# ukeSJTU/tiaozhanbei-unet

Measured on AMD Instinct MI355X. Metric: training images/sec, AnomalyUNet 256x256 bs=32 per GPU, higher is better.
Workload: dtype bf16; 1 GPU; AnomalyUNet 3x256x256, bs=32/GPU, MSE+focal loss, Adam (BASELINE.json configs[2], synthetic randn images, bernoulli masks); global_batch=32, parallelism=dp1, accumulate=fp32, master_params=fp32, dist_world=1, reserved_cus=0, cu_budget=256

## Files before the change

### tiaozhanbei_unet_amd/csrc/common.h

```cpp
#pragma once
#include <hip/hip_runtime.h>
#include <stdint.h>
#include <stdio.h>

#include "../../include/unet_hip.h"

typedef __bf16 bf16_t;
typedef __attribute__((ext_vector_type(8))) __bf16 bf16x8;
typedef __attribute__((ext_vector_type(4))) __bf16 bf16x4;
typedef __attribute__((ext_vector_type(4))) short s16x4;
typedef __attribute__((ext_vector_type(4))) float f32x4;
typedef __attribute__((ext_vector_type(16))) float f32x16;
typedef __attribute__((ext_vector_type(4))) uint32_t u32x4;
typedef __attribute__((ext_vector_type(2))) uint32_t u32x2;

#define WAVE 64

void unet_set_error(const char* fmt, ...);
int32_t unet_check_launch(const char* what);

#define UNET_REQUIRE(cond, code, ...)  \
  do {                                 \
    if (!(cond)) {                     \
      unet_set_error(__VA_ARGS__);     \
      return (code);                   \
    }                                  \
  } while (0)

int unet_cu_budget();
void unet_set_max_lds(const void* kernel, int bytes);

void unet_prof_begin(int kclass, hipStream_t s);
void unet_prof_end(int kclass, double flops, hipStream_t s, const char* kernel, double bytes);
struct ProfScope {
  int k; double f; hipStream_t s; const char* name;
  double bytes;
  ProfScope(int kclass, double flops, hipStream_t st, const char* kernel = nullptr, double alg_bytes = 0.0)
      : k(kclass), f(flops), s(st), name(kernel), bytes(alg_bytes) {
    unet_prof_begin(k, s);
  }
  ~ProfScope() { unet_prof_end(k, f, s, name, bytes); }
};

bool unet_internal_convt_gemm_ok(int mode, int dtype, int n, int h, int w, int c_in, int c_out);
int32_t unet_internal_convt_gemm(int mode, int n, int h, int w, const void* a, const void* w_packed, const float* bias,
                                 void* out, int c_in, int c_out, hipStream_t s);

int32_t unet_internal_colsum(int dtype, const void* x, int64_t pixels, int C, float* out, float* ws,
                              size_t ws_bytes, hipStream_t s);

int32_t unet_internal_bn_partials(int dtype, const void* y, int64_t pixels, int C, float* part, int* n_parts,
                                  hipStream_t s);

template <typename T> struct ET;
template <> struct ET<float> {
  static constexpr int ES = 4;
  static constexpr int PIECE = 4;
  static constexpr int KGC = 8;
  __device__ static inline float to_f(float v) { return v; }
  __device__ static inline float from_f(float v) { return v; }
};
template <> struct ET<bf16_t> {
  static constexpr int ES = 2;
  static constexpr int PIECE = 8;
  static constexpr int KGC = 16;
  __device__ static inline float to_f(bf16_t v) { return (float)v; }
  __device__ static inline bf16_t from_f(float v) { return (bf16_t)v; }
};

template <typename T> struct Vec;
template <> struct Vec<float> {
  static constexpr int N = 4;
  __device__ static inline void load(const float* p, float (&o)[4]) {
    f32x4 v = *reinterpret_cast<const f32x4*>(p);
    o[0] = v[0]; o[1] = v[1]; o[2] = v[2]; o[3] = v[3];
  }
  __device__ static inline void store(float* p, const float (&o)[4]) {
    f32x4 v = {o[0], o[1], o[2], o[3]};
    *reinterpret_cast<f32x4*>(p) = v;
  }
};
template <> struct Vec<bf16_t> {
  static constexpr int N = 8;
  __device__ static inline void load(const bf16_t* p, float (&o)[8]) {
    bf16x8 v = *reinterpret_cast<const bf16x8*>(p);
#pragma unroll
    for (int i = 0; i < 8; ++i) o[i] = (float)v[i];
  }
  __device__ static inline void store(bf16_t* p, const float (&o)[8]) {
    bf16x8 v;
#pragma unroll
    for (int i = 0; i < 8; ++i) v[i] = (bf16_t)o[i];
    *reinterpret_cast<bf16x8*>(p) = v;
  }
};

__host__ __device__ static inline int cdiv(int a, int b) { return (a + b - 1) / b; }
__host__ __device__ static inline int64_t cdiv64(int64_t a, int64_t b) { return (a + b - 1) / b; }

__device__ __forceinline__ uint32_t score_key(float x) {
  uint32_t u = __float_as_uint(x);
  if (u == 0x80000000u) u = 0u;
  return (u & 0x80000000u) ? ~u : (u | 0x80000000u);
}
__device__ __forceinline__ float score_of_key(uint32_t k) {
  return __uint_as_float((k & 0x80000000u) ? (k & 0x7fffffffu) : ~k);
}
__device__ __forceinline__ bool finite_score(float x) { return (__float_as_uint(x) & 0x7f800000u) != 0x7f800000u; }

__host__ __device__ static inline int unet_seg_col(int q, int split, int c) {
  if (split > 0 && q >= split) {
    const int p0 = (split + 63) / 64 * 64;
    if (q < p0) return -1;
    q = q - p0 + split;
  }
  return q < c ? q : -1;
}

__device__ static inline float unet_pack_seg_value(const float* __restrict__ w, int Co, int Ci, int rows, int K, int mode,
                                                   int split, long long i, const float* __restrict__ scale) {
  const int b = (int)(i % K);
  const long long t = i / K;
  const int a = (int)(t % rows), tap = (int)(t / rows);
  if (mode == UNET_PACK_CONV_FWD) {
    const int ci = unet_seg_col(b, split, Ci);
    return (a < Co && ci >= 0) ? w[((long long)a * Ci + ci) * 9 + tap] * (scale ? scale[a] : 1.f) : 0.f;
  }
  const int ci = unet_seg_col(a, split, Ci);
  return (b < Co && ci >= 0) ? w[((long long)b * Ci + ci) * 9 + (8 - tap)] : 0.f;
}
```

### tiaozhanbei_unet_amd/csrc/first.hip

```cpp
#include <stdlib.h>

#include <algorithm>

#include "conv_common.h"

namespace {

constexpr unsigned OOB = 0xFFFFFFF0u;
constexpr int FIRST_CO = 64;

struct SegPos { int seg, y, n; };
__device__ __forceinline__ SegPos seg_step(SegPos p, int dseg, int dy, int dn, int segs_row, int H) {
  p.seg += dseg;
  int c = p.seg >= segs_row;
  p.seg -= c ? segs_row : 0;
  p.y += dy + c;
  c = p.y >= H;
  p.y -= c ? H : 0;
  p.n += dn + c;
  return p;
}
struct SegWalk { SegPos first; int dseg, dy, dn; };
__device__ __forceinline__ SegWalk seg_walk(long long u0, long long stride, int segs_row, int H) {
  SegWalk w;
// ... 26 lines not shown
#pragma unroll
  for (int ct = 0; ct < 4; ++ct)
#pragma unroll
    for (int e = 0; e < 8; ++e) {
      const int k = kb * 8 + e;
      float v = 0.f;
      if (k < K) {
        const int tap = k / P.CI, ci = k - tap * P.CI;
        v = P.w[((ct * 16 + l15) * P.CI + ci) * 9 + tap];
      }
      wa[ct][e] = (bf16_t)v;
    }
  int rel[8], reli[8], dyv[8], dxv[8];
#pragma unroll
  for (int e = 0; e < 8; ++e) {
    const int k = kb * 8 + e;
    const int tap = k < K ? k / P.CI : 0, ci = k < K ? k - tap * P.CI : 0;
    dyv[e] = k < K ? tap / 3 - 1 : 1 << 20;
    dxv[e] = tap % 3 - 1;
    rel[e] = (ci * HW + dyv[e] * P.W + dxv[e]) * 4;
    reli[e] = k < K ? rel[e] : 0;
  }

  const int segs_row = P.W >> 4;
  const long long stride = (long long)gridDim.x * 4;
  const unsigned img_bytes = (unsigned)P.CI * HW * 4u;

  auto gather = [&](SegPos q, float (&xv)[8]) {
    const int x = q.seg * 16 + l15;
    const __amdgpu_buffer_rsrc_t rs =
        __builtin_amdgcn_make_buffer_rsrc((void*)(P.x + (size_t)q.n * P.CI * HW), (short)0, (int)img_bytes, 0x00020000);
    const int base = (q.y * P.W + x) * 4;
    if (q.y > 0 && q.y + 1 < P.H && q.seg > 0 && q.seg + 1 < segs_row) {
#pragma unroll
      for (int e = 0; e < 8; ++e)
        xv[e] = __builtin_bit_cast(float, __builtin_amdgcn_raw_buffer_load_b32(rs, (unsigned)(base + reli[e]), 0, 0));
    } else {
#pragma unroll
      for (int e = 0; e < 8; ++e) {
        const bool ok = (unsigned)(q.y + dyv[e]) < (unsigned)P.H && (unsigned)(x + dxv[e]) < (unsigned)P.W;
        xv[e] = __builtin_bit_cast(float, __builtin_amdgcn_raw_buffer_load_b32(rs, ok ? (unsigned)(base + rel[e]) : OOB, 0, 0));
      }
    }
  };

  float bs[4][4], bq[4][4];
#pragma unroll
  for (int ct = 0; ct < 4; ++ct)
#pragma unroll
    for (int j = 0; j < 4; ++j) { bs[ct][j] = 0.f; bq[ct][j] = 0.f; }

  constexpr int FU = 2;
  const int wave_u = __builtin_amdgcn_readfirstlane(wave);
  const SegWalk wk = seg_walk(((long long)blockIdx.x * 4 + wave_u) * FU, stride * FU, segs_row, P.H);
  SegPos cur = wk.first;
  float xc[FU][8], xn[FU][8];
#pragma unroll
  for (int i = 0; i < FU; ++i) {
    const SegPos q = seg_step(cur, i, 0, 0, segs_row, P.H);
    if (q.n < P.N) gather(q, xc[i]);
  }
  while (cur.n < P.N) {
    const SegPos nxt = seg_step(cur, wk.dseg, wk.dy, wk.dn, segs_row, P.H);
#pragma unroll
    for (int i = 0; i < FU; ++i) {
      const SegPos q = seg_step(nxt, i, 0, 0, segs_row, P.H);
      if (q.n < P.N) gather(q, xn[i]);
    }
#pragma unroll
    for (int i = 0; i < FU; ++i) {
      const SegPos q = seg_step(cur, i, 0, 0, segs_row, P.H);
      if (q.n >= P.N) break;
      bf16x8 fb;
#pragma unroll
      for (int e = 0; e < 8; ++e) fb[e] = (bf16_t)xc[i][e];
      f32x4 acc[4];
#pragma unroll
      for (int ct = 0; ct < 4; ++ct) {
        acc[ct] = f32x4{0.f, 0.f, 0.f, 0.f};
        acc[ct] = __builtin_amdgcn_mfma_f32_16x16x32_bf16(wa[ct], fb, acc[ct], 0, 0, 0);
      }
      const long long pix = ((long long)q.n * P.H + q.y) * P.W + q.seg * 16 + l15;
      bf16_t* orow = reinterpret_cast<bf16_t*>(P.y) + pix * FIRST_CO;
#pragma unroll
      for (int cp = 0; cp < 2; ++cp) {
        bf16x4 ra, rb;
#pragma unroll
        for (int j = 0; j < 4; ++j) { ra[j] = (bf16_t)acc[2 * cp][j]; rb[j] = (bf16_t)acc[2 * cp + 1][j]; }
#pragma unroll
        for (int j = 0; j < 4; ++j) {
          const float qa = (float)ra[j], qb = (float)rb[j];
          bs[2 * cp][j] += qa;      bq[2 * cp][j] = fmaf(qa, qa, bq[2 * cp][j]);
          bs[2 * cp + 1][j] += qb;  bq[2 * cp + 1][j] = fmaf(qb, qb, bq[2 * cp + 1][j]);
        }
        const u32x2 ua = __builtin_bit_cast(u32x2, ra), ub = __builtin_bit_cast(u32x2, rb);
        const auto s0 = __builtin_amdgcn_permlane16_swap(ua[0], ub[0], false, false);
        const auto s1 = __builtin_amdgcn_permlane16_swap(ua[1], ub[1], false, false);
        *reinterpret_cast<u32x4*>(orow + cp * 32 + (kb & 1) * 16 + (kb >> 1) * 8) = u32x4{s0[0], s1[0], s0[1], s1[1]};
      }
    }
#pragma unroll
    for (int i = 0; i < FU; ++i)
#pragma unroll
      for (int e = 0; e < 8; ++e) xc[i][e] = xn[i][e];
    cur = nxt;
  }

  if (P.part) {
    {
      float rv[32];
#pragma unroll
      for (int ct = 0; ct < 4; ++ct)
#pragma unroll
        for (int j = 0; j < 4; ++j) { rv[ct * 4 + j] = bs[ct][j]; rv[16 + ct * 4 + j] = bq[ct][j]; }
      row16_sum_n(rv);
#pragma unroll
      for (int ct = 0; ct < 4; ++ct)
#pragma unroll
        for (int j = 0; j < 4; ++j) { bs[ct][j] = rv[ct * 4 + j]; bq[ct][j] = rv[16 + ct * 4 + j]; }
    }
    if (l15 == 0) {
#pragma unroll
      for (int ct = 0; ct < 4; ++ct)
#pragma unroll
        for (int j = 0; j < 4; ++j) {
          red[wave][0][ct * 16 + kb * 4 + j] = bs[ct][j];
          red[wave][1][ct * 16 + kb * 4 + j] = bq[ct][j];
        }
    }
    __syncthreads();
    if (tid < 2 * FIRST_CO) {
      const int q = tid / FIRST_CO, c = tid - q * FIRST_CO;
      const float t = ((red[0][q][c] + red[1][q][c]) + red[2][q][c]) + red[3][q][c];
      P.part[((size_t)blockIdx.x * 2 + q) * FIRST_CO + c] = t;
    }
  }
}

__device__ inline bf16x8 tr_frag2(const char* base, int off0, int off1) {
  typedef __attribute__((address_space(3))) s16x4 lds_s16x4;
  s16x4 lo = __builtin_amdgcn_ds_read_tr16_b64_v4i16((lds_s16x4*)(base + off0));
  s16x4 hi = __builtin_amdgcn_ds_read_tr16_b64_v4i16((lds_s16x4*)(base + off1));
  typedef __attribute__((ext_vector_type(8))) short s16x8;
  s16x8 v = {lo[0], lo[1], lo[2], lo[3], hi[0], hi[1], hi[2], hi[3]};
  return __builtin_bit_cast(bf16x8, v);
}

template <bool BNB>
__global__ __launch_bounds__(256, BNB ? 2 : 4) void first_wgrad_kernel(const FirstParams P) {
  constexpr int SEGB = BNB ? 4096 : 2048;
  __shared__ __attribute__((aligned(16))) char smem[BNB ? 4 * 2 * 2 * 4096 : 4 * FIRST_CO * 32 * 4];
  typedef __attribute__((address_space(3))) void lds_void;
  const int tid = threadIdx.x, lane = tid & 63, wave = tid >> 6;
  const int l31 = lane & 31, hh = lane >> 5;
  const int K = 9 * P.CI;
  const int HW = P.H * P.W;
  constexpr int WU = 2;
  char* const wbuf = smem + wave * (WU * 2 * SEGB);

  const bool kvalid = l31 < K;
  const int tap = kvalid ? l31 / P.CI : 0, ci = kvalid ? l31 - tap * P.CI : 0;
  const int dy = tap / 3 - 1, dx = tap % 3 - 1;
  const int relb = (ci * HW + dy * P.W + dx + 8 * hh) * 4;

  const int g = lane >> 4, i16 = lane & 15;
  const int kq = 8 * (g >> 1) + (i16 >> 2);
  const int chb = (16 * (g & 1) + 4 * (i16 & 3)) * 2;
  const int swz = ((kq >> 1) & 1) << 2;
  int aoff[2];
#pragma unroll
  for (int wr = 0; wr < 2; ++wr) {
    const int cb = wr * 64 + chb;
    aoff[wr] = kq * 128 + ((((cb >> 4) ^ swz)) << 4) + (cb & 15);
  }
  unsigned dsrc[2];
#pragma unroll
  for (int i = 0; i < 2; ++i) {
    const int row = i * 8 + (lane >> 3), pp = lane & 7;
    dsrc[i] = (unsigned)(row * 128 + ((pp ^ (((row >> 1) & 1) << 2)) << 4));
  }

  const int segs_row = P.W >> 4;
  const long long stride = (long long)gridDim.x * 4;
  const unsigned img_bytes = (unsigned)P.CI * HW * 4u;
  const long long dy_total = (long long)P.N * HW * FIRST_CO * 2;
  auto issue = [&](SegPos q, int slot, float (&xv)[8]) {
    const int seg = q.seg, y = q.y, n = q.n;
    const long long pix0 = ((long long)n * P.H + y) * P.W + seg * 16;
    const __amdgpu_buffer_rsrc_t drs = __builtin_amdgcn_make_buffer_rsrc(
        (void*)(P.y + pix0 * (FIRST_CO * 2)), (short)0, (int)std::min<long long>(2048, dy_total - pix0 * (FIRST_CO * 2)),
        0x00020000);
#pragma unroll
    for (int i = 0; i < 2; ++i)
      __builtin_amdgcn_raw_ptr_buffer_load_lds(drs, (lds_void*)(wbuf + slot * SEGB + i * 1024), 16, dsrc[i], 0, 0, 0);
    if constexpr (BNB) {
      const __amdgpu_buffer_rsrc_t yrs = __builtin_amdgcn_make_buffer_rsrc(
          (void*)(P.y_raw + pix0 * (FIRST_CO * 2)), (short)0, (int)std::min<long long>(2048, dy_total - pix0 * (FIRST_CO * 2)),
          0x00020000);
#pragma unroll
      for (int i = 0; i < 2; ++i)
        __builtin_amdgcn_raw_ptr_buffer_load_lds(yrs, (lds_void*)(wbuf + slot * SEGB + 2048 + i * 1024), 16, dsrc[i], 0, 0, 0);
    }
    const __amdgpu_buffer_rsrc_t xrs =
        __builtin_amdgcn_make_buffer_rsrc((void*)(P.x + (size_t)n * P.CI * HW), (short)0, (int)img_bytes, 0x00020000);
    const int x0 = seg * 16;
    const int base = (y * P.W + x0) * 4 + relb;
    if (y > 0 && y + 1 < P.H && seg > 0 && seg + 1 < segs_row) {
      const unsigned b0 = kvalid ? (unsigned)base : 0u;
#pragma unroll
      for (int e = 0; e < 8; ++e)
        xv[e] = __builtin_bit_cast(float, __builtin_amdgcn_raw_buffer_load_b32(xrs, b0 + e * 4, 0, 0));
    } else {
      const bool yok = kvalid && (unsigned)(y + dy) < (unsigned)P.H;
#pragma unroll
      for (int e = 0; e < 8; ++e) {
        const bool ok = yok && (unsigned)(x0 + 8 * hh + e + dx) < (unsigned)P.W;
        xv[e] = __builtin_bit_cast(float, __builtin_amdgcn_raw_buffer_load_b32(xrs, ok ? (unsigned)(base + e * 4) : OOB, 0, 0));
      }
    }
  };

  f32x16 acc[2];
#pragma unroll
  for (int wr = 0; wr < 2; ++wr)
#pragma unroll
    for (int r = 0; r < 16; ++r) acc[wr][r] = 0.f;

  constexpr int NV = BNB ? 12 : 10;
  float cA[2], cB[2], cK[2];
  if constexpr (BNB) {
#pragma unroll
    for (int wr = 0; wr < 2; ++wr) {
      const int ch = wr * 32 + 16 * (g & 1) + i16;
      cA[wr] = P.coefs[ch]; cB[wr] = P.coefs[FIRST_CO + ch]; cK[wr] = P.coefs[2 * FIRST_CO + ch];
    }
  }
  auto issue_or_skip = [&](SegPos q, int slot, float (&xv)[8]) {
    if (q.n < P.N) {
      issue(q, slot, xv);
    } else {
      const __amdgpu_buffer_rsrc_t nul = __builtin_amdgcn_make_buffer_rsrc((void*)P.x, (short)0, 0, 0x00020000);
#pragma unroll
      for (int i = 0; i < (BNB ? 4 : 2); ++i)
        __builtin_amdgcn_raw_ptr_buffer_load_lds(nul, (lds_void*)(wbuf + slot * SEGB + i * 1024), 16, OOB, 0, 0, 0);
#pragma unroll
      for (int e = 0; e < 8; ++e) xv[e] = __builtin_bit_cast(float, __builtin_amdgcn_raw_buffer_load_b32(nul, OOB, 0, 0));
    }
  };
  const int wave_u = __builtin_amdgcn_readfirstlane(wave);
  const SegWalk wk = seg_walk(((long long)blockIdx.x * 4 + wave_u) * WU, stride * WU, segs_row, P.H);
  SegPos cur = wk.first;
  float xc[WU][8], xn[WU][8];
  int buf = 0;
#pragma unroll
  for (int i = 0; i < WU; ++i) issue_or_skip(seg_step(cur, i, 0, 0, segs_row, P.H), i, xc[i]);
  while (cur.n < P.N) {
    const SegPos nxt = seg_step(cur, wk.dseg, wk.dy, wk.dn, segs_row, P.H);
#pragma unroll
    for (int i = 0; i < WU; ++i) issue_or_skip(seg_step(nxt, i, 0, 0, segs_row, P.H), (buf ^ 1) * WU + i, xn[i]);
    asm volatile("s_waitcnt vmcnt(%0)" ::"n"(NV * WU) : "memory");
#pragma unroll
    for (int i = 0; i < WU; ++i) {
      bf16x8 fb;
#pragma unroll
      for (int e = 0; e < 8; ++e) fb[e] = (bf16_t)xc[i][e];
      const char* sb = wbuf + (buf * WU + i) * SEGB;
#pragma unroll
      for (int wr = 0; wr < 2; ++wr) {
        bf16x8 fa = tr_frag2(sb, aoff[wr], aoff[wr] + 4 * 128);
        if constexpr (BNB) {
          const bf16x8 fy = tr_frag2(sb + 2048, aoff[wr], aoff[wr] + 4 * 128);
#pragma unroll
          for (int e = 0; e < 8; ++e)
            fa[e] = (bf16_t)fmaf(cA[wr], (float)fa[e], fmaf(cB[wr], (float)fy[e], cK[wr]));
        }
        acc[wr] = __builtin_amdgcn_mfma_f32_32x32x16_bf16(fa, fb, acc[wr], 0, 0, 0);
      }
    }
#pragma unroll
    for (int i = 0; i < WU; ++i)
#pragma unroll
      for (int e = 0; e < 8; ++e) xc[i][e] = xn[i][e];
    buf ^= 1;
    cur = nxt;
  }
  asm volatile("s_waitcnt vmcnt(0)" ::: "memory");

  __syncthreads();
  float* red = reinterpret_cast<float*>(smem);
#pragma unroll
  for (int wr = 0; wr < 2; ++wr)
#pragma unroll
    for (int r = 0; r < 16; ++r) {
      const int co = wr * 32 + (r & 3) + 8 * (r >> 2) + 4 * hh;
      red[(wave * FIRST_CO + co) * 32 + l31] = acc[wr][r];
    }
  __syncthreads();
  for (int i = tid; i < FIRST_CO * 32; i += 256) {
    const float t = ((red[i] + red[FIRST_CO * 32 + i]) + red[2 * FIRST_CO * 32 + i]) + red[3 * FIRST_CO * 32 + i];
    P.part[(size_t)blockIdx.x * (FIRST_CO * 32) + i] = t;
  }
}

__global__ __launch_bounds__(256) void first_wgrad_reduce_kernel(const float* __restrict__ part, int nparts, int CI,
                                                                 float* __restrict__ dw) {
  __shared__ float red[8][32];
  const int co = blockIdx.x, k = threadIdx.x & 31, pl = threadIdx.x >> 5;
  float s0 = 0.f, s1 = 0.f;
  int b = pl;
  for (; b + 8 < nparts; b += 16) {
    s0 += part[(size_t)b * (FIRST_CO * 32) + co * 32 + k];
    s1 += part[(size_t)(b + 8) * (FIRST_CO * 32) + co * 32 + k];
  }
  if (b < nparts) s0 += part[(size_t)b * (FIRST_CO * 32) + co * 32 + k];
  red[pl][k] = s0 + s1;
  __syncthreads();
  if (threadIdx.x < 9 * CI) {
    const int kk = threadIdx.x, tap = kk / CI, ci = kk - tap * CI;
    float t = red[0][kk];
#pragma unroll
    for (int i = 1; i < 8; ++i) t += red[i][kk];
    dw[(co * CI + ci) * 9 + tap] = t;
  }
}

int first_blocks(long long units, int per_iter, int per_cu) {
  long long b = (units + 4 * per_iter - 1) / (4 * per_iter);
  return (int)std::min<long long>(b, 256 * per_cu);
}

}

extern "C" int32_t unet_conv3x3_first_supported(int32_t c_in, int32_t c_out, int32_t h, int32_t w) {
  return (c_in >= 1 && 9 * c_in <= 32 && c_out == FIRST_CO && h > 0 && w > 0 && w % 16 == 0) ? 1 : 0;
}

extern "C" int32_t unet_conv3x3_first_stats(int32_t n, int32_t h, int32_t w, const float* x, int32_t c_in,
                                            const float* weight, void* y, float* partial, int32_t* n_parts,
                                            void* stream) {
  UNET_REQUIRE(x && weight && y, UNET_ERR_BAD_ARG, "unet_conv3x3_first_stats: null pointer");
  UNET_REQUIRE(n > 0 && unet_conv3x3_first_supported(c_in, FIRST_CO, h, w), UNET_ERR_UNSUPPORTED,
               "unet_conv3x3_first_stats: n=%d c_in=%d h=%d w=%d (needs 9*c_in <= 32, w %% 16 == 0)", n, c_in, h, w);
  UNET_REQUIRE((long long)c_in * h * w * 4 < 0x7FFFFFFFLL, UNET_ERR_UNSUPPORTED, "unet_conv3x3_first_stats: image too large");
  const long long units = (long long)n * h * (w / 16);
  const int blocks = first_blocks(units, 2, 3);
  FirstParams P{x, weight, (char*)y, partial, n, c_in, h, w, nullptr, nullptr};
  hipStream_t s = (hipStream_t)stream;
  ProfScope prof(UNET_K_CONV_FWD, 2.0 * n * h * w * (double)FIRST_CO * c_in * 9, s);
  hipLaunchKernelGGL(first_fwd_kernel, dim3(blocks), dim3(256), 0, s, P);
  if (n_parts) *n_parts = partial ? blocks : 0;
  return unet_check_launch("first_fwd_kernel");
}

extern "C" size_t unet_conv3x3_first_wgrad_workspace(int32_t n, int32_t h, int32_t w) {
  const long long units = (long long)n * h * (w / 16 > 0 ? w / 16 : 1);
  return (size_t)first_blocks(units, 2, 4) * FIRST_CO * 32 * sizeof(float);
}

static int32_t first_wgrad_impl(int32_t n, int32_t h, int32_t w, const float* x, int32_t c_in, const void* dy, const void* y_raw,
                                const float* coefs, float* dw, void* workspace, size_t workspace_bytes, void* stream,
                                const char* what) {
  UNET_REQUIRE(x && dy && dw && workspace, UNET_ERR_BAD_ARG, "%s: null pointer", what);
  UNET_REQUIRE(n > 0 && unet_conv3x3_first_supported(c_in, FIRST_CO, h, w), UNET_ERR_UNSUPPORTED,
               "%s: n=%d c_in=%d h=%d w=%d", what, n, c_in, h, w);
  UNET_REQUIRE((long long)c_in * h * w * 4 < 0x7FFFFFFFLL, UNET_ERR_UNSUPPORTED, "%s: image too large", what);
  UNET_REQUIRE(workspace_bytes >= unet_conv3x3_first_wgrad_workspace(n, h, w), UNET_ERR_WORKSPACE, "%s: workspace too small", what);
  const long long units = (long long)n * h * (w / 16);
  const int blocks = first_blocks(units, 2, 4);
  FirstParams P{x, nullptr, (char*)const_cast<void*>(dy), (float*)workspace, n, c_in, h, w, (const char*)y_raw, coefs};
  hipStream_t s = (hipStream_t)stream;
  ProfScope prof(UNET_K_CONV_WGRAD, 2.0 * n * h * w * (double)FIRST_CO * c_in * 9, s);
  if (y_raw) hipLaunchKernelGGL(first_wgrad_kernel<true>, dim3(blocks), dim3(256), 0, s, P);
  else hipLaunchKernelGGL(first_wgrad_kernel<false>, dim3(blocks), dim3(256), 0, s, P);
  int32_t rc = unet_check_launch("first_wgrad_kernel");
  if (rc) return rc;
  hipLaunchKernelGGL(first_wgrad_reduce_kernel, dim3(FIRST_CO), dim3(256), 0, s, (const float*)workspace, blocks, c_in, dw);
  return unet_check_launch("first_wgrad_reduce_kernel");
}

extern "C" int32_t unet_conv3x3_first_wgrad(int32_t n, int32_t h, int32_t w, const float* x, int32_t c_in,
                                            const void* dy, float* dw, void* workspace, size_t workspace_bytes,
                                            void* stream) {
  return first_wgrad_impl(n, h, w, x, c_in, dy, nullptr, nullptr, dw, workspace, workspace_bytes, stream,
                          "unet_conv3x3_first_wgrad");
}

extern "C" int32_t unet_conv3x3_first_wgrad_bn(int32_t n, int32_t h, int32_t w, const float* x, int32_t c_in,
                                               const void* dz, const void* y, const float* coefs, float* dw,
                                               void* workspace, size_t workspace_bytes, void* stream) {
  UNET_REQUIRE(y && coefs, UNET_ERR_BAD_ARG, "unet_conv3x3_first_wgrad_bn: null pointer");
  return first_wgrad_impl(n, h, w, x, c_in, dz, y, coefs, dw, workspace, workspace_bytes, stream,
                          "unet_conv3x3_first_wgrad_bn");
}
```

### tiaozhanbei_unet_amd/csrc/wgrad.hip

```cpp
#include <stdlib.h>

#include <algorithm>

#include "common.h"

namespace {

struct WView { const char* p; int C, H, W, oy, ox; };

#ifdef PDMA_STAMPS
void* g_wgrad_debug = nullptr;
#endif
struct WgradParams {
  void* debug;
  WView rt;
  WView ct[2];
  int N, H, W;
  int Crow, Ccol;
  float* partial;
  int split, tilesPerSplit, tilesX, tilesY, nR, nC;
  int xcd_chunk;
};

__device__ inline bool wgrad_block_coords(const WgradParams& P, int& sp, int& rtile, int& ctile) {
// ... 671 lines not shown
                  a3 = p[(size_t)(k + 12) * slab];
      s += a0; s += a1; s += a2; s += a3;
    }
    for (; k < split; k += 4) s += p[(size_t)k * slab];
  }
  red[ks][cl] = s;
  __syncthreads();
  if (ks == 0 && c < cols_out)
    out[((size_t)r * cols_out + c) * TAPS + tap] = (red[0][cl] + red[1][cl]) + (red[2][cl] + red[3][cl]);
}

struct Plan { int tilesX, tilesY, nR, nC, split, tilesPerSplit; size_t bytes; };

template <int TAPS>
Plan make_plan(int n, int h, int w, int crow, int ccol) {
  Plan p;
  constexpr int TH = (TAPS == 9) ? 8 : 4;
  p.tilesX = cdiv(w, 16);
  p.tilesY = cdiv(h, TH);
  p.nR = crow / 64;
  p.nC = ccol / 64;
  const long long ntiles = (long long)n * p.tilesY * p.tilesX;
  long long want = 2LL * unet_cu_budget() / ((long long)p.nR * p.nC);
  if (want < 1) want = 1;
  if (want > ntiles) want = ntiles;
  p.tilesPerSplit = (int)cdiv64(ntiles, want);
  p.split = (int)cdiv64(ntiles, p.tilesPerSplit);
  p.bytes = (size_t)p.split * TAPS * crow * ccol * sizeof(float);
  return p;
}

inline Plan make_plan16(int n, int h, int w, int crow, int ccol) {
  Plan p;
  const bool paired = w <= 16;
  p.tilesX = paired ? 1 : cdiv(w, 32);
  p.tilesY = cdiv(h, 4);
  p.nR = crow / 128;
  p.nC = ccol / 64;
  const long long ntiles = (long long)(paired ? (n + 1) / 2 : n) * p.tilesY * p.tilesX;
  long long want = (long long)unet_cu_budget() / ((long long)p.nR * p.nC);
  if (want < 1) want = 1;
  if (want > ntiles) want = ntiles;
  p.tilesPerSplit = (int)cdiv64(ntiles, want);
  p.split = (int)cdiv64(ntiles, p.tilesPerSplit);
  p.bytes = (size_t)p.split * 9 * crow * ccol * sizeof(float);
  return p;
}

template <bool PAIRED>
void launch16(const WgradParams& P, long long blocks, hipStream_t s) {
  using C = W16<PAIRED>;
  auto kern = wgrad16_kernel<PAIRED>;
  unet_set_max_lds(reinterpret_cast<const void*>(kern), C::LDS);
  hipLaunchKernelGGL(kern, dim3((unsigned)blocks), dim3(512), C::LDS, s, P);
}

template <typename T, int TAPS>
int32_t run(WgradParams& P, const Plan& pl, float* out, int rows_out, int cols_out, int kclass, hipStream_t s) {
  P.tilesX = pl.tilesX; P.tilesY = pl.tilesY; P.nR = pl.nR; P.nC = pl.nC;
  P.split = pl.split; P.tilesPerSplit = pl.tilesPerSplit;
  long long blocks = (long long)pl.split * pl.nR * pl.nC;
  P.xcd_chunk = 0;
  if (blocks >= 16) {
    P.xcd_chunk = (int)cdiv64(blocks, 8);
    blocks = 8LL * P.xcd_chunk;
  }
  const double flops = 2.0 * P.N * P.H * P.W * (double)P.Crow * P.Ccol * TAPS;
  int split_used = pl.split;
  {
    const double alg_bytes = (double)P.N * P.H * P.W * ((double)P.Crow + P.Ccol * (TAPS == 9 ? 1.0 : 4.0)) * sizeof(T) +
                             4.0 * TAPS * rows_out * cols_out;
    constexpr bool DMA = sizeof(T) == 2 && TAPS == 9;
    const bool v16 = DMA && P.Crow % 128 == 0;
    ProfScope prof(kclass, flops, s,
                   v16 ? "wgrad16_kernel (+ reduce)" : (DMA ? "wgrad_dma_kernel (+ reduce)" : "wgrad_kernel (+ reduce)"), alg_bytes);
    if constexpr (DMA) {
      if (v16) {
        const Plan p16 = make_plan16(P.N, P.H, P.W, P.Crow, P.Ccol);
        P.tilesX = p16.tilesX; P.tilesY = p16.tilesY; P.nR = p16.nR; P.nC = p16.nC;
        P.split = p16.split; P.tilesPerSplit = p16.tilesPerSplit;
        split_used = p16.split;
        long long b16 = (long long)p16.split * p16.nR * p16.nC;
        P.xcd_chunk = 0;
        if (b16 >= 16) { P.xcd_chunk = (int)cdiv64(b16, 8); b16 = 8LL * P.xcd_chunk; }
        if (P.W <= 16) launch16<true>(P, b16, s);
        else launch16<false>(P, b16, s);
      } else {
        unet_set_max_lds(reinterpret_cast<const void*>(wgrad_dma_kernel), WDma::LDS);
        hipLaunchKernelGGL(wgrad_dma_kernel, dim3((unsigned)blocks), dim3(256), WDma::LDS, s, P);
      }
    } else {
      using C = WCfg<T, TAPS>;
      auto kern = wgrad_kernel<T, TAPS>;
      unet_set_max_lds(reinterpret_cast<const void*>(kern), C::LDS);
      hipLaunchKernelGGL(kern, dim3((unsigned)blocks), dim3(256), C::LDS, s, P);
    }
    int32_t rc = unet_check_launch("wgrad_kernel");
    if (rc) return rc;
    if (split_used >= 16) {
      const long long rb = (long long)rows_out * ((cols_out + 63) / 64) * TAPS;
      hipLaunchKernelGGL(wgrad_reduce_wide_kernel<TAPS>, dim3((unsigned)rb), dim3(256), 0, s, (const float*)P.partial,
                         out, split_used, P.Crow, P.Ccol, rows_out, cols_out);
    } else {
      const long long total = (long long)rows_out * cols_out;
      const int rb = (int)std::min<long long>(cdiv64(total, 256), 4096);
      hipLaunchKernelGGL(wgrad_reduce_kernel<TAPS>, dim3(rb), dim3(256), 0, s, (const float*)P.partial, out, split_used,
                         P.Crow, P.Ccol, rows_out, cols_out);
    }
  }
  return unet_check_launch("wgrad_reduce_kernel");
}

inline int pad64(int c) { return (c + 63) / 64 * 64; }

}

extern "C" size_t unet_conv3x3_wgrad_workspace(int32_t n, int32_t h, int32_t w, int32_t c_in, int32_t c_out) {
  size_t bytes = make_plan<9>(n, h, w, pad64(c_out), pad64(c_in)).bytes;
  if (pad64(c_out) % 128 == 0)
    bytes = std::max(bytes, make_plan16(n, h, w, pad64(c_out), pad64(c_in)).bytes);
  return bytes;
}

extern "C" int32_t unet_conv3x3_wgrad(int32_t dtype, int32_t n, int32_t h, int32_t w, const unet_view src[2],
                                      const void* dy, int32_t c_out, float* dw, int32_t c_in_param,
                                      void* workspace, size_t workspace_bytes, void* stream) {
  UNET_REQUIRE(src && src[0].ptr && dy && dw && workspace, UNET_ERR_BAD_ARG, "unet_conv3x3_wgrad: null pointer");
  UNET_REQUIRE(n > 0 && h > 0 && w > 0, UNET_ERR_BAD_ARG, "unet_conv3x3_wgrad: bad dims");
  const int ctot = src[0].c + (src[1].ptr ? src[1].c : 0);
  UNET_REQUIRE(c_out % 64 == 0, UNET_ERR_UNSUPPORTED, "unet_conv3x3_wgrad: c_out %d not a multiple of 64", c_out);
  UNET_REQUIRE(ctot % 64 == 0 && (!src[1].ptr || src[0].c % 64 == 0), UNET_ERR_UNSUPPORTED,
               "unet_conv3x3_wgrad: input channels %d(+%d) must be multiples of 64", src[0].c,
               src[1].ptr ? src[1].c : 0);
  UNET_REQUIRE(c_in_param <= ctot, UNET_ERR_BAD_ARG, "unet_conv3x3_wgrad: c_in_param %d > %d", c_in_param, ctot);
  const Plan pl = make_plan<9>(n, h, w, c_out, ctot);
  const size_t need = unet_conv3x3_wgrad_workspace(n, h, w, ctot, c_out);
  UNET_REQUIRE(workspace_bytes >= need, UNET_ERR_WORKSPACE, "unet_conv3x3_wgrad: workspace %zu < %zu", workspace_bytes, need);
  WgradParams P{};
#ifdef PDMA_STAMPS
  P.debug = g_wgrad_debug;
#endif
  P.rt = WView{(const char*)dy, c_out, h, w, 0, 0};
  P.ct[0] = WView{(const char*)src[0].ptr, src[0].c, src[0].h, src[0].w, src[0].off_y, src[0].off_x};
  P.ct[1] = src[1].ptr ? WView{(const char*)src[1].ptr, src[1].c, src[1].h, src[1].w, src[1].off_y, src[1].off_x}
                       : WView{nullptr, 0, 0, 0, 0, 0};
  P.N = n; P.H = h; P.W = w;
  P.Crow = c_out; P.Ccol = ctot;
  P.partial = (float*)workspace;
  hipStream_t s = (hipStream_t)stream;
  if (dtype == UNET_BF16) return run<bf16_t, 9>(P, pl, dw, c_out, c_in_param, UNET_K_CONV_WGRAD, s);
  if (dtype == UNET_F32) return run<float, 9>(P, pl, dw, c_out, c_in_param, UNET_K_CONV_WGRAD, s);
  unet_set_error("unet_conv3x3_wgrad: dtype %d", dtype);
  return UNET_ERR_BAD_ARG;
}

namespace {

struct CtwParams {
  const char* x; const char* dy; float* part;
  int N, H, W, tiles, tiles_per_split;
};
template <int CIN>
struct CfgCTW {
  static constexpr int COUT = CIN / 2, NC = 2 * CIN;
  static constexpr int TP = 32;
  static constexpr int X_BYTES = TP * 256, D_BYTES = TP * 512, BUF = X_BYTES + D_BYTES;
  static constexpr int NDMA = BUF / 1024 / 4;
  static constexpr int RB = CIN / 128, CB = NC / 256;
  static constexpr int LDS = 2 * BUF;
};

template <int CIN>
__global__ __launch_bounds__(256, 2) void convt_wgrad_ws_kernel(const CtwParams P) {
  using C = CfgCTW<CIN>;
  extern __shared__ __attribute__((aligned(16))) char smem[];
  typedef __attribute__((address_space(3))) void lds_void;
  const int tid = threadIdx.x, lane = tid & 63, wave = tid >> 6;
  const int wr = wave & 1, wc = wave >> 1;
  const int l31 = lane & 31, hh = lane >> 5;
  const int rb = blockIdx.y / C::CB, cb = blockIdx.y % C::CB;
  const int sp = blockIdx.x;
  const int t_begin = sp * P.tiles_per_split, t_end = min(t_begin + P.tiles_per_split, P.tiles);

  f32x16 acc[2][4];
#pragma unroll
  for (int a = 0; a < 2; ++a)
#pragma unroll
    for (int b = 0; b < 4; ++b)
#pragma unroll
      for (int r = 0; r < 16; ++r) acc[a][b][r] = 0.f;
  float cs[4] = {0.f, 0.f, 0.f, 0.f};

  const int g = lane >> 4, i16 = lane & 15;
  const int kq = 8 * (g >> 1) + (i16 >> 2);
  const int chb = (16 * (g & 1) + 4 * (i16 & 3)) * 2;
  const int swz = (kq & 3) << 2;
  int aoff[2], boff[4];
#pragma unroll
  for (int mt = 0; mt < 2; ++mt) {
    const int c = (wr * 64 + mt * 32) * 2 + chb;
    aoff[mt] = kq * 256 + (((c >> 4) ^ swz) << 4) + (c & 15);
  }
#pragma unroll
  for (int nt = 0; nt < 4; ++nt) {
    const int c = (wc * 128 + nt * 32) * 2 + chb;
    boff[nt] = C::X_BYTES + kq * 512 + (((c >> 4) ^ swz) << 4) + (c & 15);
  }

  int d_row[C::NDMA];
  unsigned d_off[C::NDMA];
#pragma unroll
  for (int j = 0; j < C::NDMA; ++j) {
    const int ii = j * 4 + wave;
    if (ii < 8) {
      const int row = ii * 4 + (lane >> 4), piece = lane & 15;
      d_row[j] = row;
      d_off[j] = (unsigned)(rb * 256 + ((piece ^ ((row & 3) << 2)) << 4));
    } else {
      const int row = (ii - 8) * 2 + (lane >> 5), piece = lane & 31;
      const int n0 = cb * 256 + ((piece ^ ((row & 3) << 2)) << 3);
      const int z = n0 / C::COUT, co = n0 - z * C::COUT;
      d_row[j] = row;
      d_off[j] = (unsigned)(z | (co << 8));
    }
  }
  const long long x_total = (long long)P.N * P.H * P.W * CIN * 2;
  const long long dy_total = 2 * x_total;
  const __amdgpu_buffer_rsrc_t xrs = __builtin_amdgcn_make_buffer_rsrc(
      (void*)P.x, (short)0, (int)std::min<long long>(x_total, 0x7FFFFFFFLL), 0x00020000);
  const __amdgpu_buffer_rsrc_t drs = __builtin_amdgcn_make_buffer_rsrc(
      (void*)P.dy, (short)0, (int)std::min<long long>(dy_total, 0x7FFFFFFFLL), 0x00020000);
  const bool narrow = P.W < C::TP;
  const int tiles_row = narrow ? 1 : P.W / C::TP;

  auto dma = [&](int tile, int buf) {
    const int ry = narrow ? tile * 2 : tile / tiles_row;
    const int x0 = narrow ? 0 : (tile - ry * tiles_row) * C::TP;
    const int n = ry / P.H, y = ry - n * P.H;
    const long long xpix0 = (long long)ry * P.W + x0;
    const long long dpix0 = ((long long)n * 2 * P.H + 2 * y) * (2 * P.W) + 2 * x0;
#pragma unroll
    for (int j = 0; j < C::NDMA; ++j) {
      const int ii = j * 4 + wave;
      char* dst = smem + buf * C::BUF + ii * 1024;
      if (ii < 8) {
        const unsigned vo = (unsigned)((xpix0 + d_row[j]) * (CIN * 2)) + d_off[j];
        __builtin_amdgcn_raw_ptr_buffer_load_lds(xrs, (lds_void*)dst, 16, vo, 0, 0, 0);
      } else {
        const int z = d_off[j] & 255, co = d_off[j] >> 8;
        const int rr = narrow ? (d_row[j] >> 4) * (4 * P.W) + 2 * (d_row[j] & 15) : 2 * d_row[j];
        const long long dp = dpix0 + (long long)(z >> 1) * (2 * P.W) + rr + (z & 1);
        const unsigned vo = (unsigned)(dp * (C::COUT * 2) + co * 2);
        __builtin_amdgcn_raw_ptr_buffer_load_lds(drs, (lds_void*)dst, 16, vo, 0, 0, 0);
      }
    }
  };

  if (t_begin < t_end) dma(t_begin, 0);
  for (int tile = t_begin; tile < t_end; ++tile) {
    const int buf = (tile - t_begin) & 1;
    asm volatile("s_waitcnt vmcnt(0)" ::: "memory");
    __builtin_amdgcn_s_barrier();
    if (tile + 1 < t_end) dma(tile + 1, buf ^ 1);
    const char* sb = smem + buf * C::BUF;
#pragma unroll
    for (int ks = 0; ks < C::TP / 16; ++ks) {
      bf16x8 fa[2], fb[4];
#pragma unroll
      for (int mt = 0; mt < 2; ++mt) fa[mt] = tr_frag2(sb, aoff[mt] + ks * 16 * 256, aoff[mt] + ks * 16 * 256 + 4 * 256);
#pragma unroll
      for (int nt = 0; nt < 4; ++nt) fb[nt] = tr_frag2(sb, boff[nt] + ks * 16 * 512, boff[nt] + ks * 16 * 512 + 4 * 512);
      if (wr == 0 && rb == 0) {
#pragma unroll
        for (int nt = 0; nt < 4; ++nt)
#pragma unroll
          for (int e = 0; e < 8; ++e) cs[nt] += (float)fb[nt][e];
      }
#pragma unroll
      for (int mt = 0; mt < 2; ++mt)
#pragma unroll
        for (int nt = 0; nt < 4; ++nt)
          acc[mt][nt] = __builtin_amdgcn_mfma_f32_32x32x16_bf16(fa[mt], fb[nt], acc[mt][nt], 0, 0, 0);
    }
  }

  float* slab = P.part + (size_t)sp * (CIN + 1) * C::NC;
#pragma unroll
  for (int nt = 0; nt < 4; ++nt) {
    const int col = cb * 256 + wc * 128 + nt * 32 + l31;
#pragma unroll
    for (int mt = 0; mt < 2; ++mt)
#pragma unroll
      for (int r = 0; r < 16; ++r) {
        const int row = rb * 128 + wr * 64 + mt * 32 + (r & 3) + 8 * (r >> 2) + 4 * hh;
        slab[(size_t)row * C::NC + col] = acc[mt][nt][r];
      }
    if (wr == 0 && rb == 0) {
      const float t = cs[nt] + __shfl_xor(cs[nt], 32);
      if (hh == 0) slab[(size_t)CIN * C::NC + col] = t;
    }
  }
}

__global__ __launch_bounds__(256) void convt_wgrad_ws_reduce_kernel(const float* __restrict__ part, int nsplit, int CIN,
                                                                    float* __restrict__ dw, float* __restrict__ db) {
  __shared__ float red[4][64];
  const int NC = 2 * CIN, COUT = CIN / 2;
  const int row = blockIdx.x, c = threadIdx.x & 63, sl = threadIdx.x >> 6;
  const size_t stride = (size_t)(CIN + 1) * NC;
  float s0 = 0.f, s1 = 0.f;
  if (row < CIN) {
    const int col = blockIdx.y * 64 + c;
    const float* p = part + (size_t)row * NC + col;
    int s = sl;
    for (; s + 4 < nsplit; s += 8) { s0 += p[(size_t)s * stride]; s1 += p[(size_t)(s + 4) * stride]; }
    if (s < nsplit) s0 += p[(size_t)s * stride];
  } else {
    const int co = blockIdx.y * 64 + c;
    if (co < COUT) {
      const float* p = part + (size_t)CIN * NC + co;
      for (int s = sl; s < nsplit; s += 4) {
        const float* q = p + (size_t)s * stride;
        s0 += ((q[0] + q[COUT]) + q[2 * COUT]) + q[3 * COUT];
      }
    }
  }
  red[sl][c] = s0 + s1;
  __syncthreads();
  if (sl == 0) {
    const float t = ((red[0][c] + red[1][c]) + red[2][c]) + red[3][c];
    if (row < CIN) {
      const int col = blockIdx.y * 64 + c;
      const int z = col / COUT, co = col - z * COUT;
      dw[((size_t)row * COUT + co) * 4 + z] = t;
    } else if (blockIdx.y * 64 + c < COUT) {
      db[blockIdx.y * 64 + c] = t;
    }
  }
}

template <int CIN>
int32_t launch_convt_wgrad_ws(const void* x, const void* dy, int n, int h, int w, float* dw, float* db, void* workspace,
                              size_t workspace_bytes, hipStream_t s) {
  using C = CfgCTW<CIN>;
  const long long px = (long long)n * h * w;
  CtwParams P{(const char*)x, (const char*)dy, (float*)workspace, n, h, w, (int)(px / C::TP), 0};
  const int yb = C::RB * C::CB;
  int nsplit = 2 * unet_cu_budget() / yb;
  if (nsplit < 1) nsplit = 1;
  if (nsplit > P.tiles) nsplit = P.tiles;
  P.tiles_per_split = (P.tiles + nsplit - 1) / nsplit;
  nsplit = (P.tiles + P.tiles_per_split - 1) / P.tiles_per_split;
  const size_t need = (size_t)nsplit * (CIN + 1) * C::NC * sizeof(float);
  UNET_REQUIRE(workspace_bytes >= need, UNET_ERR_WORKSPACE, "unet_convt2x2_wgrad: workspace %zu < %zu", workspace_bytes, need);
  auto kern = convt_wgrad_ws_kernel<CIN>;
  unet_set_max_lds(reinterpret_cast<const void*>(kern), C::LDS);
  {
    ProfScope prof(UNET_K_CONVT_WGRAD, 2.0 * px * 4.0 * C::COUT * CIN, s, "convt_wgrad_ws_kernel (+ reduce)");
    hipLaunchKernelGGL(kern, dim3(nsplit, yb), dim3(256), C::LDS, s, P);
    int32_t rc = unet_check_launch("convt_wgrad_ws_kernel");
    if (rc) return rc;
    hipLaunchKernelGGL(convt_wgrad_ws_reduce_kernel, dim3(CIN + 1, C::NC / 64), dim3(256), 0, s, (const float*)workspace,
                       nsplit, CIN, dw, db);
  }
  return unet_check_launch("convt_wgrad_ws_reduce_kernel");
}

inline bool convt_wgrad_ws_ok(int dtype, int n, int h, int w, int c_in, int c_out) {
  const long long xb = (long long)n * h * w * c_in * 2;
  return dtype == UNET_BF16 && (c_in == 128 || c_in == 256 || c_in == 512 || c_in == 1024) && c_out * 2 == c_in &&
         (w % 32 == 0 || (w == 16 && h % 2 == 0)) && ((long long)n * h * w) % 32 == 0 &&
         2 * xb < 0x7FFFFFFFLL;
}
inline size_t convt_wgrad_ws_bytes(int n, int h, int w, int c_in) {
  const long long tiles = (long long)n * h * w / 32;
  const int yb = (c_in / 128) * (c_in / 128);
  long long nsplit = 2 * unet_cu_budget() / yb;
  if (nsplit < 1) nsplit = 1;
  if (nsplit > tiles) nsplit = tiles;
  return (size_t)nsplit * (c_in + 1) * (2 * c_in) * sizeof(float);
}

}

extern "C" size_t unet_convt2x2_wgrad_workspace(int32_t n, int32_t h, int32_t w, int32_t c_in, int32_t c_out) {
  size_t bytes = make_plan<4>(n, h, w, pad64(c_in), pad64(c_out)).bytes;
  if (convt_wgrad_ws_ok(UNET_BF16, n, h, w, c_in, c_out)) bytes = std::max(bytes, convt_wgrad_ws_bytes(n, h, w, c_in));
  return bytes;
}

extern "C" int32_t unet_convt2x2_wgrad(int32_t dtype, int32_t n, int32_t h, int32_t w, const void* x,
                                       int32_t c_in, const void* dy, int32_t c_out, float* dw, float* db,
                                       void* workspace, size_t workspace_bytes, void* stream) {
  UNET_REQUIRE(x && dy && dw && db && workspace, UNET_ERR_BAD_ARG, "unet_convt2x2_wgrad: null pointer");
  UNET_REQUIRE(n > 0 && h > 0 && w > 0, UNET_ERR_BAD_ARG, "unet_convt2x2_wgrad: bad dims");
  UNET_REQUIRE(c_in % 64 == 0 && c_out % 64 == 0, UNET_ERR_UNSUPPORTED,
               "unet_convt2x2_wgrad: channels %d -> %d must be multiples of 64", c_in, c_out);
  if (convt_wgrad_ws_ok(dtype, n, h, w, c_in, c_out)) {
    hipStream_t st = (hipStream_t)stream;
    if (c_in == 128) return launch_convt_wgrad_ws<128>(x, dy, n, h, w, dw, db, workspace, workspace_bytes, st);
    if (c_in == 256) return launch_convt_wgrad_ws<256>(x, dy, n, h, w, dw, db, workspace, workspace_bytes, st);
    if (c_in == 512) return launch_convt_wgrad_ws<512>(x, dy, n, h, w, dw, db, workspace, workspace_bytes, st);
    return launch_convt_wgrad_ws<1024>(x, dy, n, h, w, dw, db, workspace, workspace_bytes, st);
  }
  const Plan pl = make_plan<4>(n, h, w, c_in, c_out);
  UNET_REQUIRE(workspace_bytes >= pl.bytes, UNET_ERR_WORKSPACE, "unet_convt2x2_wgrad: workspace %zu < %zu",
               workspace_bytes, pl.bytes);
  WgradParams P{};
  P.rt = WView{(const char*)x, c_in, h, w, 0, 0};
  P.ct[0] = WView{(const char*)dy, c_out, 2 * h, 2 * w, 0, 0};
  P.ct[1] = WView{nullptr, 0, 0, 0, 0, 0};
  P.N = n; P.H = h; P.W = w;
  P.Crow = c_in; P.Ccol = c_out;
  P.partial = (float*)workspace;
  hipStream_t s = (hipStream_t)stream;
  int32_t rc;
  if (dtype == UNET_BF16) rc = run<bf16_t, 4>(P, pl, dw, c_in, c_out, UNET_K_CONVT_WGRAD, s);
  else if (dtype == UNET_F32) rc = run<float, 4>(P, pl, dw, c_in, c_out, UNET_K_CONVT_WGRAD, s);
  else { unet_set_error("unet_convt2x2_wgrad: dtype %d", dtype); return UNET_ERR_BAD_ARG; }
  if (rc) return rc;
  return unet_internal_colsum(dtype, dy, (int64_t)n * 4 * h * w, c_out, db, (float*)workspace, workspace_bytes, s);
}

#ifdef PDMA_STAMPS
extern "C" void unet_debug_set_buffer_wgrad(void* p) { g_wgrad_debug = p; }
#endif
```

Before: 1782 images/sec.

## Vectorize and software-pipeline split-K partial reductions for wgrad kernels

After: 1787 images/sec, median of 6. No clear change (+0.3%).

```diff
diff --git a/tiaozhanbei_unet_amd/csrc/common.h b/tiaozhanbei_unet_amd/csrc/common.h
--- a/tiaozhanbei_unet_amd/csrc/common.h
+++ b/tiaozhanbei_unet_amd/csrc/common.h
@@ -98,6 +98,42 @@
 __host__ __device__ static inline int cdiv(int a, int b) { return (a + b - 1) / b; }
 __host__ __device__ static inline int64_t cdiv64(int64_t a, int64_t b) { return (a + b - 1) / b; }
 
+template <int U>
+__device__ __forceinline__ void slab_batch4(f32x4& s, const float* __restrict__& q, size_t inc) {
+  f32x4 a[U];
+#pragma unroll
+  for (int u = 0; u < U; ++u) a[u] = *reinterpret_cast<const f32x4*>(q + u * inc);
+#pragma unroll
+  for (int u = 0; u < U; ++u) s += a[u];
+  q += U * inc;
+}
+template <int UMAX>
+__device__ __forceinline__ f32x4 slab_sum4(const float* __restrict__ p, size_t stride, int k, int step, int n) {
+  f32x4 s = {0.f, 0.f, 0.f, 0.f};
+  int m = k < n ? (n - k + step - 1) / step : 0;
+  const float* __restrict__ q = p + (size_t)k * stride;
+  const size_t inc = (size_t)step * stride;
+  if (m >= UMAX) {
+    f32x4 a[UMAX];
+#pragma unroll
+    for (int u = 0; u < UMAX; ++u) a[u] = *reinterpret_cast<const f32x4*>(q + u * inc);
+    for (q += UMAX * inc, m -= UMAX; m >= UMAX; q += UMAX * inc, m -= UMAX) {
+#pragma unroll
+      for (int u = 0; u < UMAX; ++u) {
+        s += a[u];
+        a[u] = *reinterpret_cast<const f32x4*>(q + u * inc);
+      }
+    }
+#pragma unroll
+    for (int u = 0; u < UMAX; ++u) s += a[u];
+  }
+  if constexpr (UMAX > 8) if (m & 8) slab_batch4<8>(s, q, inc);
+  if constexpr (UMAX > 4) if (m & 4) slab_batch4<4>(s, q, inc);
+  if (m & 2) slab_batch4<2>(s, q, inc);
+  if (m & 1) slab_batch4<1>(s, q, inc);
+  return s;
+}
+
 __device__ __forceinline__ uint32_t score_key(float x) {
   uint32_t u = __float_as_uint(x);
   if (u == 0x80000000u) u = 0u;
diff --git a/tiaozhanbei_unet_amd/csrc/first.hip b/tiaozhanbei_unet_amd/csrc/first.hip
--- a/tiaozhanbei_unet_amd/csrc/first.hip
+++ b/tiaozhanbei_unet_amd/csrc/first.hip
@@ -352,25 +352,20 @@
   }
 }
 
-__global__ __launch_bounds__(256) void first_wgrad_reduce_kernel(const float* __restrict__ part, int nparts, int CI,
+__global__ __launch_bounds__(128) void first_wgrad_reduce_kernel(const float* __restrict__ part, int nparts, int CI,
                                                                  float* __restrict__ dw) {
-  __shared__ float red[8][32];
-  const int co = blockIdx.x, k = threadIdx.x & 31, pl = threadIdx.x >> 5;
-  float s0 = 0.f, s1 = 0.f;
-  int b = pl;
-  for (; b + 8 < nparts; b += 16) {
-    s0 += part[(size_t)b * (FIRST_CO * 32) + co * 32 + k];
-    s1 += part[(size_t)(b + 8) * (FIRST_CO * 32) + co * 32 + k];
-  }
-  if (b < nparts) s0 += part[(size_t)b * (FIRST_CO * 32) + co * 32 + k];
-  red[pl][k] = s0 + s1;
+  __shared__ float red[16][32];
+  const int co = blockIdx.x, c4 = threadIdx.x & 7, lane = threadIdx.x >> 3;
+  const f32x4 s = slab_sum4<16>(part + co * 32 + 4 * c4, (size_t)FIRST_CO * 32, lane, 16, nparts);
+#pragma unroll
+  for (int e = 0; e < 4; ++e) red[lane][4 * c4 + e] = s[e];
   __syncthreads();
   if (threadIdx.x < 9 * CI) {
-    const int kk = threadIdx.x, tap = kk / CI, ci = kk - tap * CI;
-    float t = red[0][kk];
-#pragma unroll
-    for (int i = 1; i < 8; ++i) t += red[i][kk];
-    dw[(co * CI + ci) * 9 + tap] = t;
+    const int o = threadIdx.x, ci = o / 9, tap = o - ci * 9, kk = tap * CI + ci;
+    float t = red[0][kk] + red[8][kk];
+#pragma unroll
+    for (int i = 1; i < 8; ++i) t += red[i][kk] + red[i + 8][kk];
+    dw[co * 9 * CI + o] = t;
   }
 }
 
@@ -424,7 +419,7 @@
   else hipLaunchKernelGGL(first_wgrad_kernel<false>, dim3(blocks), dim3(256), 0, s, P);
   int32_t rc = unet_check_launch("first_wgrad_kernel");
   if (rc) return rc;
-  hipLaunchKernelGGL(first_wgrad_reduce_kernel, dim3(FIRST_CO), dim3(256), 0, s, (const float*)workspace, blocks, c_in, dw);
+  hipLaunchKernelGGL(first_wgrad_reduce_kernel, dim3(FIRST_CO), dim3(128), 0, s, (const float*)workspace, blocks, c_in, dw);
   return unet_check_launch("first_wgrad_reduce_kernel");
 }
 
diff --git a/tiaozhanbei_unet_amd/csrc/wgrad.hip b/tiaozhanbei_unet_amd/csrc/wgrad.hip
--- a/tiaozhanbei_unet_amd/csrc/wgrad.hip
+++ b/tiaozhanbei_unet_amd/csrc/wgrad.hip
@@ -997,39 +997,60 @@
   }
 }
 
-__global__ __launch_bounds__(256) void convt_wgrad_ws_reduce_kernel(const float* __restrict__ part, int nsplit, int CIN,
-                                                                    float* __restrict__ dw, float* __restrict__ db) {
-  __shared__ float red[4][64];
+constexpr int CTR_CO = 32, CTR_LD = CTR_CO + 1, CTR_BIAS_CO = 4, CTR_BIAS_SPLITS = 512;
+template <int UMAX>
+__global__ __launch_bounds__(256) __attribute__((amdgpu_waves_per_eu(UMAX > 8 ? 3 : 6)))
+void convt_wgrad_ws_reduce_kernel(const float* __restrict__ part, int nsplit, int CIN, float* __restrict__ dw,
+                                  float* __restrict__ db) {
+  __shared__ float red[8 * 4 * CTR_LD];
+  __shared__ __attribute__((aligned(16))) float tz[CTR_BIAS_SPLITS * CTR_BIAS_CO];
   const int NC = 2 * CIN, COUT = CIN / 2;
-  const int row = blockIdx.x, c = threadIdx.x & 63, sl = threadIdx.x >> 6;
   const size_t stride = (size_t)(CIN + 1) * NC;
-  float s0 = 0.f, s1 = 0.f;
-  if (row < CIN) {
-    const int col = blockIdx.y * 64 + c;
-    const float* p = part + (size_t)row * NC + col;
-    int s = sl;
-    for (; s + 4 < nsplit; s += 8) { s0 += p[(size_t)s * stride]; s1 += p[(size_t)(s + 4) * stride]; }
-    if (s < nsplit) s0 += p[(size_t)s * stride];
-  } else {
-    const int co = blockIdx.y * 64 + c;
-    if (co < COUT) {
-      const float* p = part + (size_t)CIN * NC + co;
-      for (int s = sl; s < nsplit; s += 4) {
-        const float* q = p + (size_t)s * stride;
-        s0 += ((q[0] + q[COUT]) + q[2 * COUT]) + q[3 * COUT];
-      }
-    }
-  }
-  red[sl][c] = s0 + s1;
-  __syncthreads();
-  if (sl == 0) {
-    const float t = ((red[0][c] + red[1][c]) + red[2][c]) + red[3][c];
-    if (row < CIN) {
-      const int col = blockIdx.y * 64 + c;
-      const int z = col / COUT, co = col - z * COUT;
-      dw[((size_t)row * COUT + co) * 4 + z] = t;
-    } else if (blockIdx.y * 64 + c < COUT) {
-      db[blockIdx.y * 64 + c] = t;
+  const int t = threadIdx.x;
+  const int nbias = COUT / CTR_BIAS_CO, nchunk = COUT / CTR_CO;
+  const long long items = nbias + (long long)CIN * nchunk;
+  for (long long item = blockIdx.x; item < items; item += gridDim.x) {
+    if (item < nbias) {
+      const int co0 = (int)item * CTR_BIAS_CO;
+      const int sl = t / CTR_BIAS_CO, c = t % CTR_BIAS_CO;
+      float s0 = 0.f;
+      for (int sb = 0; sb < nsplit; sb += CTR_BIAS_SPLITS) {
+        const int ns = min(CTR_BIAS_SPLITS, nsplit - sb);
+#pragma unroll 2
+        for (int i = t; i < ns * (CTR_BIAS_CO / 4); i += 256) {
+          const int sp = i / (CTR_BIAS_CO / 4), c4 = i % (CTR_BIAS_CO / 4);
+          const float* q = part + (size_t)(sb + sp) * stride + (size_t)CIN * NC + co0 + 4 * c4;
+          const f32x4 q0 = *reinterpret_cast<const f32x4*>(q), q1 = *reinterpret_cast<const f32x4*>(q + COUT),
+                      q2 = *reinterpret_cast<const f32x4*>(q + 2 * COUT), q3 = *reinterpret_cast<const f32x4*>(q + 3 * COUT);
+          *reinterpret_cast<f32x4*>(tz + sp * CTR_BIAS_CO + 4 * c4) = ((q0 + q1) + q2) + q3;
+        }
+        __syncthreads();
+        if (t < 4 * CTR_BIAS_CO) {
+#pragma unroll 8
+          for (int sp = sl; sp < ns; sp += 4) s0 += tz[sp * CTR_BIAS_CO + c];
+        }
+        __syncthreads();
+      }
+      if (t < 4 * CTR_BIAS_CO) red[t] = s0 + 0.f;
+      __syncthreads();
+      if (t < CTR_BIAS_CO)
+        db[co0 + t] = ((red[t] + red[CTR_BIAS_CO + t]) + red[2 * CTR_BIAS_CO + t]) + red[3 * CTR_BIAS_CO + t];
+      __syncthreads();
+    } else {
+      const long long m = item - nbias;
+      const int row = (int)(m / nchunk), co0 = (int)(m % nchunk) * CTR_CO;
+      const int c4 = t & 7, z = (t >> 3) & 3, l8 = t >> 5;
+      const f32x4 s = slab_sum4<UMAX>(part + (size_t)row * NC + z * COUT + co0 + 4 * c4, stride, l8, 8, nsplit);
+      float* q = red + (l8 * 4 + z) * CTR_LD + 4 * c4;
+      q[0] = s[0]; q[1] = s[1]; q[2] = s[2]; q[3] = s[3];
+      __syncthreads();
+      if (t < 4 * CTR_CO) {
+        constexpr int L = 4 * CTR_LD;
+        const float* v = red + (t & 3) * CTR_LD + (t >> 2);
+        const float r0 = v[0] + v[4 * L], r1 = v[L] + v[5 * L], r2 = v[2 * L] + v[6 * L], r3 = v[3 * L] + v[7 * L];
+        dw[((size_t)row * COUT + co0) * 4 + t] = ((r0 + r1) + r2) + r3;
+      }
+      __syncthreads();
     }
   }
 }
@@ -1055,8 +1076,14 @@
     hipLaunchKernelGGL(kern, dim3(nsplit, yb), dim3(256), C::LDS, s, P);
     int32_t rc = unet_check_launch("convt_wgrad_ws_kernel");
     if (rc) return rc;
-    hipLaunchKernelGGL(convt_wgrad_ws_reduce_kernel, dim3(CIN + 1, C::NC / 64), dim3(256), 0, s, (const float*)workspace,
-                       nsplit, CIN, dw, db);
+    const long long items = C::COUT / CTR_BIAS_CO + (long long)CIN * (C::COUT / CTR_CO);
+    const unsigned grid = (unsigned)std::min<long long>(items, 8LL * unet_cu_budget());
+    if (nsplit > 32)
+      hipLaunchKernelGGL(convt_wgrad_ws_reduce_kernel<16>, dim3(grid), dim3(256), 0, s, (const float*)workspace, nsplit,
+                         CIN, dw, db);
+    else
+      hipLaunchKernelGGL(convt_wgrad_ws_reduce_kernel<4>, dim3(grid), dim3(256), 0, s, (const float*)workspace, nsplit,
+                         CIN, dw, db);
   }
   return unet_check_launch("convt_wgrad_ws_reduce_kernel");
 }
```
